# ajzhai/PEANUT

Measured on AMD Instinct MI355X. Metric: maps/sec for 480x480x(4+N_cat) prediction fwd, batch 32, higher is better.
Workload: dtype f32; 1 GPU; 480x480, 14-channel (4+10) partial maps -> 6-class prediction forward (PSPNet R50-V1c-D8), batch 32 per GPU, seeded random-init weights; survey_config=2, global_batch=32, parallelism=dp1 (map shards, no data-path collective)

## Files before the change

peanut_amd/csrc/conv_pw_ares.hip:

```cpp
#include <stdlib.h>

#include "common.h"
#include "conv_common.h"

namespace peanut {

namespace {

typedef const __attribute__((address_space(1))) void* gptr_t;
typedef __attribute__((address_space(3))) void* lptr_t;

__device__ __forceinline__ float load_uncounted(const float* ptr) {
  float v;
  asm volatile("global_load_dword %0, %1, off" : "=v"(v) : "v"(ptr) : "memory");
  return v;
}
template <int CH>
__device__ __forceinline__ void wait_uncounted(const float (&r)[CH], float a, float b) {
  static_assert(CH == 4 || CH == 8, "chunk of 4 or 8 values");
  __builtin_amdgcn_sched_barrier(0);
  if constexpr (CH == 4)
    asm volatile("s_waitcnt vmcnt(0)" ::"v"(r[0]), "v"(r[1]), "v"(r[2]), "v"(r[3]), "v"(a), "v"(b) : "memory");
  else
    asm volatile("s_waitcnt vmcnt(0)" ::"v"(r[0]), "v"(r[1]), "v"(r[2]), "v"(r[3]), "v"(r[4]), "v"(r[5]), "v"(r[6]), "v"(r[7]), "v"(a), "v"(b)
                 : "memory");
  __builtin_amdgcn_sched_barrier(0);
}

template <int NK, bool FLUSH>
__global__ __launch_bounds__(512) void conv_pw_ares_kernel(const ConvKParams p) {
  constexpr int BK = 32, K = NK * BK, TILE = 128 * BK;
  constexpr int CH = 32 / NK;
  static_assert(NK == 4 || NK == 8, "K = 128 or 256");
  __shared__ __attribute__((aligned(1024))) float smem[(NK + 2) * TILE];
  float* const bst = smem + NK * TILE;

  const int tid = threadIdx.x, lane = tid & 63;
  const int wave = __builtin_amdgcn_readfirstlane(tid >> 6);
  const int lr = lane >> 3, lp = lane & 7;
  const int wm = wave >> 2, wn = wave & 3;
  const int li = lane & 31, hi = lane >> 5;
  const bool late = p.phase_shift && wave >= 4;

  const int G = gridDim.x, bid = blockIdx.x;
  const int lw = (bid & 7) * (G >> 3) + (bid >> 3);
  const int NT = p.ntiles;
  const long long U = (long long)p.mtiles * NT;
  const int u0 = (int)(U * lw / G), u1 = (int)(U * (lw + 1) / G);
  if (u0 >= u1) return;

  const int pbn = p.ares_pbn;
  unsigned a_off[2], b_off[2];
#pragma unroll
  for (int j = 0; j < 2; ++j) {
    const int r = (wave * 2 + j) * 8 + lr;
    const int c = lp ^ ((r >> 1) & 7);
    a_off[j] = r * K + c * 4;
    b_off[j] = (r / pbn) * (NK * pbn * BK) + (r % pbn) * BK + c * 4;
  }
  auto dma_a = [&](int mt, int s) {
    const float* base = p.x + (size_t)mt * (128 * K) + s * BK;
#pragma unroll
    for (int j = 0; j < 2; ++j)
      __builtin_amdgcn_global_load_lds((gptr_t)(base + a_off[j]), (lptr_t)(smem + s * TILE + (wave * 2 + j) * 256), 16, 0, 0);
  };
  auto dma_b = [&](int mt, int nt, int kt, int stage) {
    const float* base = p.w + (p.mt_per_group ? (size_t)(mt / p.mt_per_group) * p.w_group_stride : 0) + (size_t)nt * (128 * K) + kt * (pbn * BK);
#pragma unroll
    for (int j = 0; j < 2; ++j)
      __builtin_amdgcn_global_load_lds((gptr_t)(base + b_off[j]), (lptr_t)(bst + stage * TILE + (wave * 2 + j) * 256), 16, 0, 0);
  };

  const int swz = (li >> 1) & 7;
  int sw[4];
#pragma unroll
  for (int ks = 0; ks < 4; ++ks) sw[ks] = ((ks * 2 + hi) ^ swz) * 4;
  const int a_row = (wm * 64 + li) * BK;
  const int b_row = (wn * 32 + li) * BK;

  f32x16 acc[2], acc2[2], prev[2];
#pragma unroll
  for (int t = 0; t < 2; ++t)
#pragma unroll
    for (int r = 0; r < 16; ++r) { acc[t][r] = 0.f; acc2[t][r] = 0.f; prev[t][r] = 0.f; }

  const size_t lane_el = (size_t)(wm * 64 + 4 * hi) * p.cout + wn * 32 + li;
  const bool has_res = p.res != nullptr;
  const size_t rstride = has_res ? (size_t)p.cout : 0;
  const size_t ostride = (size_t)p.cout;
  const float* res_run = has_res ? p.res + lane_el : p.zeros;
  float* out_run = p.y + lane_el;
  const float* prev_sc = p.scale + wn * 32 + li;
  const float* prev_sh = p.shift + wn * 32 + li;
  bool prev_valid = false;
  float scv = 1.f, shv = 0.f;
  const float alpha = p.alpha;
  const bool relu = p.relu != 0;

#define ARES_CHUNK_LOADS(kt)                                                              \
  float resv[CH];                                                                         \
  if ((kt) == 0) {                                                                        \
    scv = load_uncounted(prev_sc);                                                        \
    shv = load_uncounted(prev_sh);                                                        \
  }                                                                                       \
  _Pragma("unroll") for (int i = 0; i < CH; ++i)                                          \
    resv[i] = load_uncounted(res_run + (size_t)(8 * (i >> 2) + (i & 3)) * rstride);       \
  res_run += (size_t)(2 * CH) * rstride;
#define ARES_CHUNK_FINISH(kt)                                                             \
  if (prev_valid) {                                                   \
    _Pragma("unroll") for (int i = 0; i < CH; ++i) {                                      \
      const int idx = (kt) * CH + i;                                                      \
      float v = prev[idx >> 4][idx & 15] * (scv * alpha) + shv;                           \
      v += resv[i];                                                                       \
      if (relu) v = relu_keep_nan(v);                                                     \
      out_run[(size_t)(8 * (i >> 2) + (i & 3)) * ostride] = v;                            \
    }                                                                                     \
  }                                                                                       \
  out_run += (size_t)(2 * CH) * ostride;

  {
    const int mt = u0 / NT, nt = u0 - mt * NT;
#pragma unroll
    for (int s = 0; s < NK; ++s) dma_a(mt, s);
    dma_b(mt, nt, 0, 0);
    asm volatile("s_waitcnt vmcnt(0)" ::: "memory");
    __builtin_amdgcn_s_barrier();
    asm volatile("" ::: "memory");
  }

  int stage = 0;
  for (int u = u0; u < u1; ++u) {
    const int mt = u / NT, nt = u - mt * NT;
    const bool nxt = u + 1 < u1;
    const int mt_n = nxt ? (u + 1) / NT : mt;
    const int nt_n = nxt ? (u + 1) - mt_n * NT : 0;
    const bool refill_next = nxt && mt_n != mt;

    static_for<NK>([&](auto kc) {
      constexpr int kt = decltype(kc)::value;
      const float* const cur_b = bst + stage * TILE;
      const float* const cur_a = smem + kt * TILE;
      const bool more = (kt + 1 < NK) || nxt;
      ARES_CHUNK_LOADS(kt)
      auto request = [&]() {
        if (more) {
          if (kt + 1 < NK) dma_b(mt, nt, kt + 1, stage ^ 1);
          else dma_b(mt_n, nt_n, 0, stage ^ 1);
        }
      };
      if (!late) request();
      __builtin_amdgcn_sched_barrier(0);
      f32x4 af[4][2], bf[4];
#pragma unroll
      for (int j = 0; j < 4; ++j) {
        af[j][0] = *reinterpret_cast<const f32x4*>(cur_a + a_row + sw[j]);
        af[j][1] = *reinterpret_cast<const f32x4*>(cur_a + a_row + 32 * BK + sw[j]);
        bf[j] = *reinterpret_cast<const f32x4*>(cur_b + b_row + sw[j]);
      }
#pragma unroll
      for (int j = 0; j < 2; ++j)
#pragma unroll
        for (int kk = 0; kk < 4; ++kk)
#pragma unroll
          for (int t = 0; t < 2; ++t) acc[t] = __builtin_amdgcn_mfma_f32_32x32x2f32(af[j][t][kk], bf[j][kk], acc[t], 0, 0, 0);
      __builtin_amdgcn_sched_barrier(0);
      if (late) request();
      __builtin_amdgcn_sched_barrier(0);
#pragma unroll
      for (int j = 2; j < 4; ++j)
#pragma unroll
        for (int kk = 0; kk < 4; ++kk)
#pragma unroll
          for (int t = 0; t < 2; ++t) acc[t] = __builtin_amdgcn_mfma_f32_32x32x2f32(af[j][t][kk], bf[j][kk], acc[t], 0, 0, 0);
      if (FLUSH && (kt & 1)) {
#pragma unroll
        for (int t = 0; t < 2; ++t) {
          acc2[t] += acc[t];
#pragma unroll
          for (int r = 0; r < 16; ++r) acc[t][r] = 0.f;
        }
      }
      wait_uncounted<CH>(resv, scv, shv);
      ARES_CHUNK_FINISH(kt)
      if (kt >= 1) { if (refill_next) dma_a(mt_n, kt - 1); }
      asm volatile("s_waitcnt lgkmcnt(0)" ::: "memory");
      __builtin_amdgcn_s_barrier();
      asm volatile("" ::: "memory");
      stage ^= 1;
    });

#pragma unroll
    for (int t = 0; t < 2; ++t) {
      prev[t] = FLUSH ? acc2[t] : acc[t];
#pragma unroll
      for (int r = 0; r < 16; ++r) { acc[t][r] = 0.f; acc2[t][r] = 0.f; }
    }
    {
      const size_t unit_el = (size_t)mt * 128 * p.cout + (size_t)nt * 128 + lane_el;
      res_run = has_res ? p.res + unit_el : p.zeros;
      out_run = p.y + unit_el;
      const int ss_off = (p.mt_per_group && p.ss_group_stride) ? (mt / p.mt_per_group) * p.ss_group_stride : 0;
      prev_sc = p.scale + ss_off + nt * 128 + wn * 32 + li;
      prev_sh = p.shift + ss_off + nt * 128 + wn * 32 + li;
      prev_valid = true;
    }
    if (refill_next) dma_a(mt_n, NK - 1);
  }

  static_for<NK>([&](auto kc) {
    constexpr int kt = decltype(kc)::value;
    ARES_CHUNK_LOADS(kt)
    wait_uncounted<CH>(resv, scv, shv);
    ARES_CHUNK_FINISH(kt)
  });
#undef ARES_CHUNK_LOADS
#undef ARES_CHUNK_FINISH
}

template <int NK, bool FLUSH>
int launch_ares_t(ConvKParams p, hipStream_t stream) {
  const int cus = device_cus();
  if (cus < 8) return fail(-3, "conv_pw_ares: no current device");
  const long long U = (long long)p.mtiles * p.ntiles;
  long long G = U < cus ? U : cus;
  G -= G % 8;
  if (G < 8) return fail(-2, "conv_pw_ares: launch too small");
  hipLaunchKernelGGL((conv_pw_ares_kernel<NK, FLUSH>), dim3((unsigned)G), dim3(512), 0, stream, p);
  hipError_t e = hipGetLastError();
  if (e != hipSuccess) return fail(-3, std::string("conv_pw_ares launch: ") + hipGetErrorString(e));
  return 0;
}

}

bool conv_pw_uses_ares(int cin, int cout, long long M, int stride, bool two_source, int flush_ktiles, int bn_tile) {
  const bool on = opt(OPT_PW_ARES) != 0;
  const long long min_units = opt(OPT_PW_ARES_MINUNITS);
  if (!on || two_source || (cin != 128 && cin != 256) || stride != 1 || M % 128 != 0 || cout % 128 != 0) return false;
  if (bn_tile != 64 && bn_tile != 128) return false;
  if (flush_ktiles != 0 && flush_ktiles != 2) return false;
  return (M / 128) * (cout / 128) >= min_units;
}

int launch_conv_pw_ares(const ConvKParams& p0, int bn_tile, hipStream_t stream) {
  ConvKParams p = p0;
  p.phase_shift = opt(OPT_PW256_PHASE) != 0;
  p.ares_pbn = bn_tile;
  p.mtiles = p.M / 128;
  p.ntiles = p.cout / 128;
  const bool flush = p.flush == 2;
  if (p.c1 == 256) return flush ? launch_ares_t<8, true>(p, stream) : launch_ares_t<8, false>(p, stream);
  return flush ? launch_ares_t<4, true>(p, stream) : launch_ares_t<4, false>(p, stream);
}

}
```

peanut_amd/csrc/conv_pw256p.hip:

```cpp
#include <stdlib.h>

#include "common.h"
#include "conv_common.h"

namespace peanut {

namespace {

typedef const __attribute__((address_space(1))) void* gptr_t;
typedef __attribute__((address_space(3))) void* lptr_t;

__device__ __forceinline__ float p_load_uncounted(const float* base, unsigned byte_off) {
  float v;
  asm volatile("s_nop 4\n\tglobal_load_dword %0, %1, %2" : "=v"(v) : "v"(byte_off), "s"(base) : "memory");
  return v;
}
template <int N>
__device__ __forceinline__ void p_wait(const float (&r)[8], float a, float b, float c, float d) {
  __builtin_amdgcn_sched_barrier(0);
  if constexpr (N == 6)
    asm volatile("s_waitcnt vmcnt(6)" ::"v"(r[0]), "v"(r[1]), "v"(r[2]), "v"(r[3]), "v"(r[4]), "v"(r[5]), "v"(r[6]), "v"(r[7]), "v"(a), "v"(b),
                 "v"(c), "v"(d)
                 : "memory");
  else
    asm volatile("s_waitcnt vmcnt(0)" ::"v"(r[0]), "v"(r[1]), "v"(r[2]), "v"(r[3]), "v"(r[4]), "v"(r[5]), "v"(r[6]), "v"(r[7]), "v"(a), "v"(b),
                 "v"(c), "v"(d)
                 : "memory");
  __builtin_amdgcn_sched_barrier(0);
}

struct PItem { int mt, nt, kt0, kt1, part; };

template <bool RAGGED, bool FLUSH>
__global__ __launch_bounds__(512) void conv_pw_glds256p_kernel(const ConvKParams p) {
  constexpr int BM = 256, BN = 128, BK = 32, WN = 2;
  constexpr int A_FLOATS = BM * BK, B_FLOATS = BN * BK, STAGE = A_FLOATS + B_FLOATS;
  constexpr int A_INSTR = 4, B_INSTR = 2;
  __shared__ __attribute__((aligned(1024))) float smem[3 * STAGE + kMaxItems * 8];
  int* const plan = reinterpret_cast<int*>(smem + 3 * STAGE);

  const int tid = threadIdx.x, lane = tid & 63;
  const int wave = __builtin_amdgcn_readfirstlane(tid >> 6);
  const int lr = lane >> 3, lp = lane & 7;
  const int wm = wave / WN, wn = wave % WN;
  const int li = lane & 31, hi = lane >> 5;
  const bool late = p.phase_shift && wave >= 4;

  const int G = gridDim.x, bid = blockIdx.x;
  const int lw = (bid & 7) * (G >> 3) + (bid >> 3);
  const int nf = p.n_full / G;
  const int sp0 = (int)((long long)p.n_sp * lw / G), sp1 = (int)((long long)p.n_sp * (lw + 1) / G);
  const long long skU = p.sk_units;
  const int u0 = (skU > 0 && lw < p.sk_g) ? (int)(skU * lw / p.sk_g) : 0, u1 = (skU > 0 && lw < p.sk_g) ? (int)(skU * (lw + 1) / p.sk_g) : 0;
  const int upt = skU > 0 ? p.nkt / p.sk_q : 1;
  const int n_frag = u1 > u0 ? (u1 - 1) / upt - u0 / upt + 1 : 0;
  const int n_items = nf + (skU > 0 ? n_frag : sp1 - sp0);
  if (n_items == 0) return;
  if (n_items > kMaxItems) __builtin_trap();
  if (tid < n_items) {
    const int i = tid;
    PItem it;
    int tile;
    if (i >= nf && skU > 0) {
      const int j = u0 / upt + (i - nf);
      const int t0 = j * upt;
      it.kt0 = ((u0 > t0 ? u0 : t0) - t0) * p.sk_q;
      it.kt1 = ((u1 < t0 + upt ? u1 : t0 + upt) - t0) * p.sk_q;
      it.part = j * p.sk_maxp + (lw - sk_owner(skU, p.sk_g, (long long)t0));
      tile = p.n_full + j;
    } else if (i < nf) {
      tile = p.p_order ? (lw / (G >> 3)) * (nf * (G >> 3)) + i * (G >> 3) + lw % (G >> 3) : lw * nf + i;
      it.kt0 = 0; it.kt1 = p.nkt; it.part = -1;
    } else {
      const int s = sp0 + (i - nf);
      const int j = s / p.split_p, part = s - j * p.split_p;
      tile = p.n_full + j;
      it.part = s;
      it.kt0 = (int)((long long)part * p.nkt / p.split_p);
      it.kt1 = (int)((long long)(part + 1) * p.nkt / p.split_p);
    }
    tile_to_mn(p, tile, &it.mt, &it.nt);
    int* e = plan + i * 8;
    e[0] = it.mt; e[1] = it.nt; e[2] = it.kt0; e[3] = it.kt1; e[4] = it.part;
  }
  __syncthreads();
  auto item_at = [&](int i) {
    const int* e = plan + i * 8;
    PItem it;
    it.mt = __builtin_amdgcn_readfirstlane(e[0]);
    it.nt = __builtin_amdgcn_readfirstlane(e[1]);
    it.kt0 = __builtin_amdgcn_readfirstlane(e[2]);
    it.kt1 = __builtin_amdgcn_readfirstlane(e[3]);
    it.part = __builtin_amdgcn_readfirstlane(e[4]);
    return it;
  };

  unsigned a_pix[A_INSTR], a_chunk[A_INSTR], b_off[B_INSTR];
#pragma unroll
  for (int j = 0; j < A_INSTR; ++j) {
    const int r = (wave * A_INSTR + j) * 8 + lr;
    a_chunk[j] = (unsigned)((lp ^ ((r >> 1) & 7)) * 16);
    a_pix[j] = 0;
  }
#pragma unroll
  for (int j = 0; j < B_INSTR; ++j) {
    const int r = (wave * B_INSTR + j) * 8 + lr;
    b_off[j] = (unsigned)(r * BK * 4 + (lp ^ ((r >> 1) & 7)) * 16);
  }
  int d_item = 0, d_left = 0, d_kt = 0;
  const float* d_wtile = p.w;
  auto cursor_open = [&](int i) {
    const PItem it = item_at(i);
    const int m0 = it.mt * BM;
#pragma unroll
    for (int j = 0; j < A_INSTR; ++j) {
      int m = m0 + (wave * A_INSTR + j) * 8 + lr;
      if (RAGGED) m = m < p.M ? m : p.M - 1;
      const int b = m / p.HoWo;
      const int rem = m - b * p.HoWo;
      const int oy = rem / p.Wo, ox = rem - oy * p.Wo;
      a_pix[j] = (unsigned)(b * p.H * p.W + oy * p.stride * p.W + ox * p.stride);
    }
    d_wtile = p.w + (p.mt_per_group ? (size_t)(it.mt / p.mt_per_group) * p.w_group_stride : 0) + (size_t)it.nt * p.nkt * (BN * BK);
    d_kt = it.kt0;
    d_left = it.kt1 - it.kt0;
  };
  const int k1 = p.c1 / BK;
  auto request = [&](float* stage) {
    const bool live = d_left > 0;
    if (!live) --d_kt;
    const bool second = d_kt >= k1;
    const char* abase = reinterpret_cast<const char*>(second ? p.x2 : p.x) + (size_t)(second ? d_kt - k1 : d_kt) * (BK * 4);
    const unsigned cbytes = (unsigned)(second ? p.c2 : p.c1) * 4u;
#pragma unroll
    for (int j = 0; j < A_INSTR; ++j)
      __builtin_amdgcn_global_load_lds((gptr_t)(abase + (a_pix[j] * cbytes + a_chunk[j])), (lptr_t)(stage + (wave * A_INSTR + j) * 256), 16, 0, 0);
    const char* bbase = reinterpret_cast<const char*>(d_wtile + (size_t)d_kt * (BN * BK));
#pragma unroll
    for (int j = 0; j < B_INSTR; ++j)
      __builtin_amdgcn_global_load_lds((gptr_t)(bbase + b_off[j]), (lptr_t)(stage + A_FLOATS + (wave * B_INSTR + j) * 256), 16, 0, 0);
    ++d_kt;
    if (live) --d_left;
  };
  auto cursor_advance = [&]() {
    if (d_left == 0 && d_item + 1 < n_items) {
      ++d_item;
      cursor_open(d_item);
    }
  };

  const int swz = (li >> 1) & 7;
  int sw[4];
#pragma unroll
  for (int ks = 0; ks < 4; ++ks) sw[ks] = ((ks * 2 + hi) ^ swz) * 4;
  const int a_row = (wm * 64 + li) * BK;
  const int b_row = A_FLOATS + (wn * 64 + li) * BK;

  f32x16 acc[2][2], prev[2][2], acc2[2][2];
#pragma unroll
  for (int t = 0; t < 2; ++t)
#pragma unroll
    for (int u = 0; u < 2; ++u)
#pragma unroll
      for (int r = 0; r < 16; ++r) { acc[t][u][r] = 0.f; prev[t][u][r] = 0.f; acc2[t][u][r] = 0.f; }
#define P256_PREV(t, u, r) (FLUSH ? acc2[t][u][r] : prev[t][u][r])
#define P256_FLUSH_STEP()                                                                                 \
  if (FLUSH) {                                                                                            \
    _Pragma("unroll") for (int t = 0; t < 2; ++t)                                                         \
      _Pragma("unroll") for (int u = 0; u < 2; ++u) {                                                     \
        acc2[t][u] += acc[t][u];                                                                          \
        _Pragma("unroll") for (int r = 0; r < 16; ++r) acc[t][u][r] = 0.f;                                \
      }                                                                                                   \
  }

  const int cout = p.cout;
  bool prev_valid = false, prev_raw = false;
  const float* prev_res = p.zeros;
  float* prev_out = p.y;
  const float* prev_ss = p.scale;
  unsigned prev_rs = 0;
  unsigned prev_os = (unsigned)cout * 4;
  int prev_rows = BM;
  const unsigned lane_row = (unsigned)(wm * 64 + 4 * hi), lane_col = (unsigned)(wn * 64 + li);
  const unsigned ss_lane = lane_col * 4;
  const unsigned shift_delta = (unsigned)((p.shift - p.scale) * 4);
  float sc0 = 1.f, sc1 = 1.f, sh0 = 0.f, sh1 = 0.f;
  const bool has_res = p.res != nullptr;
  const float alpha = p.alpha;
  const bool relu = p.relu != 0;

#define P256_EPI_SS_LOADS()                                                                                       \
  {                                                                                                               \
    sc0 = p_load_uncounted(prev_ss, ss_lane);                                                                     \
    sc1 = p_load_uncounted(prev_ss, ss_lane + 128);                                                               \
    sh0 = p_load_uncounted(prev_ss, ss_lane + shift_delta);                                                       \
    sh1 = p_load_uncounted(prev_ss, ss_lane + shift_delta + 128);                                                 \
  }
#define P256_EPI_LOADS(c)                                                                                         \
  float resv[8];                                                                                                  \
  {                                                                                                               \
    if ((c) == 0) {                                                                                               \
      sc0 = p_load_uncounted(prev_ss, ss_lane);                                                                   \
      sc1 = p_load_uncounted(prev_ss, ss_lane + 128);                                                             \
      sh0 = p_load_uncounted(prev_ss, ss_lane + shift_delta);                                                     \
      sh1 = p_load_uncounted(prev_ss, ss_lane + shift_delta + 128);                                               \
    }                                                                                                             \
    const unsigned lane_off = (lane_row * prev_rs) + (prev_rs ? lane_col * 4 : 0);                                \
                                                      \
    int row_limit = prev_rows - 1;                                                                                \
    if (RAGGED) asm volatile("" : "+s"(row_limit));                                                               \
    _Pragma("unroll") for (int i = 0; i < 8; ++i) {                                                               \
      const int r = ((c) & 1) * 8 + i, row = ((c) >> 2) * 32 + (r & 3) + 8 * (r >> 2);                            \
      unsigned roff = lane_off + (unsigned)row * prev_rs;                                                         \
      if (RAGGED) {                                                                                               \
        const int rr = (int)lane_row + row;                                                                       \
                                           \
        roff = __umul24((unsigned)(rr < row_limit ? rr : row_limit), prev_rs) + (prev_rs ? lane_col * 4 : 0);     \
      }                                                                                                           \
      resv[i] = p_load_uncounted(prev_res, roff + (prev_rs ? (((c) >> 1) & 1) * 128u : 0u));                      \
    }                                                                                                             \
  }
#define P256_EPI_FINISH(c) P256_EPI_FINISH_RV(c, resv)
#define P256_EPI_FINISH_RV(c, RV)                                                                                 \
  if (prev_valid) {                                                                                               \
    const float scv = (((c) >> 1) & 1) ? sc1 : sc0, shv = (((c) >> 1) & 1) ? sh1 : sh0;                           \
    char* const obase = reinterpret_cast<char*>(prev_out) + (lane_row * prev_os + lane_col * 4 + (((c) >> 1) & 1) * 128u); \
    _Pragma("unroll") for (int i = 0; i < 8; ++i) {                                                               \
      const int r = ((c) & 1) * 8 + i, row = ((c) >> 2) * 32 + (r & 3) + 8 * (r >> 2);                            \
      float v = P256_PREV((c) >> 2, ((c) >> 1) & 1, r);                                                           \
      if (!prev_raw) {                                                                                            \
        v = v * (scv * alpha) + shv;                                                                              \
        v += RV[i];                                                                                               \
        if (relu) v = relu_keep_nan(v);                                                                           \
      }                                                                                                           \
      if (!RAGGED || (int)lane_row + row < prev_rows) *reinterpret_cast<float*>(obase + (unsigned)row * prev_os) = v; \
    }                                                                                                             \
  }

  cursor_open(0);
  request(smem);
  cursor_advance();
  request(smem + STAGE);
  cursor_advance();
  asm volatile("s_waitcnt vmcnt(6)" ::: "memory");
  asm volatile("s_waitcnt lgkmcnt(0)" ::: "memory");
  __builtin_amdgcn_s_barrier();
  asm volatile("" ::: "memory");
  int o_cur = 0, o_mid = STAGE, o_fill = 2 * STAGE;

#define P256_MFMA_PAIR()                                                                                  \
  _Pragma("unroll") for (int j = 0; j < 2; ++j)                                                           \
    _Pragma("unroll") for (int kk = 0; kk < 4; ++kk)                                                      \
      _Pragma("unroll") for (int t = 0; t < 2; ++t)                                                       \
        _Pragma("unroll") for (int u = 0; u < 2; ++u)                                                     \
          acc[t][u] = __builtin_amdgcn_mfma_f32_32x32x2f32(af[j][t][kk], bf[j][u][kk], acc[t][u], 0, 0, 0);
#define P256_READ_PAIR(g)                                                                                            \
  _Pragma("unroll") for (int j = 0; j < 2; ++j) {                                                                    \
    _Pragma("unroll") for (int t = 0; t < 2; ++t) af[j][t] = *reinterpret_cast<const f32x4*>(cur + a_row + t * 32 * BK + sw[(g) + j]); \
    _Pragma("unroll") for (int u = 0; u < 2; ++u) bf[j][u] = *reinterpret_cast<const f32x4*>(cur + b_row + u * 32 * BK + sw[(g) + j]); \
  }
#define P256_ITERATION()                                                                                  \
  {                                                                                                       \
    const float* const cur = smem + o_cur;                                                                \
    float* const fill = smem + o_fill;                                                                    \
    float resv_none[8] = {0.f, 0.f, 0.f, 0.f, 0.f, 0.f, 0.f, 0.f};                                        \
    (void)resv_none;                                                                                      \
    P256_EPI_LOADS_IF                                                                                     \
    if (!late) request(fill);                                                                             \
    __builtin_amdgcn_sched_barrier(0);                                                                    \
    f32x4 af[2][2], bf[2][2];                                                                             \
    P256_READ_PAIR(0);                                                                                    \
    P256_MFMA_PAIR();                                                                                     \
    __builtin_amdgcn_sched_barrier(0);                                                                    \
    if (late) request(fill);                                                                              \
    __builtin_amdgcn_sched_barrier(0);                                                                    \
    P256_READ_PAIR(2);                                                                                    \
    P256_MFMA_PAIR();                                                                                     \
    p_wait<6>(P256_RESV, sc0, sc1, sh0, sh1);                                                             \
    P256_EPI_FINISH_IF                                                                                    \
    P256_FLUSH_IF                                                                                         \
    cursor_advance();                                                                                     \
    asm volatile("s_waitcnt lgkmcnt(0)" ::: "memory");                                                    \
    __builtin_amdgcn_s_barrier();                                                                         \
    asm volatile("" ::: "memory");                                                                        \
    { const int tmp = o_cur; o_cur = o_mid; o_mid = o_fill; o_fill = tmp; }                               \
  }

  for (int ci = 0; ci < n_items; ++ci) {
    const PItem it = item_at(ci);
    const int nk = it.kt1 - it.kt0;
    static_for<8>([&](auto kc) {
      constexpr int c = decltype(kc)::value;
      if (c < nk) {
        if constexpr (!FLUSH) {
#define P256_EPI_LOADS_IF P256_EPI_LOADS(c)
#define P256_EPI_FINISH_IF P256_EPI_FINISH(c)
#define P256_FLUSH_IF
#define P256_RESV resv
          P256_ITERATION()
#undef P256_EPI_LOADS_IF
#undef P256_EPI_FINISH_IF
#undef P256_FLUSH_IF
#undef P256_RESV
        } else {
#define P256_EPI_LOADS_IF if (c == 0) P256_EPI_SS_LOADS()
#define P256_EPI_FINISH_IF                                                                   \
  if (c == 0) { P256_EPI_FINISH_RV(0, resv_none) P256_EPI_FINISH_RV(1, resv_none) P256_EPI_FINISH_RV(2, resv_none) P256_EPI_FINISH_RV(3, resv_none) } \
  if (c == 1) {                                                                              \
    P256_EPI_FINISH_RV(4, resv_none) P256_EPI_FINISH_RV(5, resv_none) P256_EPI_FINISH_RV(6, resv_none) P256_EPI_FINISH_RV(7, resv_none) \
    _Pragma("unroll") for (int t = 0; t < 2; ++t)                                            \
      _Pragma("unroll") for (int u = 0; u < 2; ++u)                                          \
        _Pragma("unroll") for (int r = 0; r < 16; ++r) acc2[t][u][r] = 0.f;                  \
  }
#define P256_FLUSH_IF if (c & 1) { P256_FLUSH_STEP() }
#define P256_RESV resv_none
          P256_ITERATION()
#undef P256_EPI_LOADS_IF
#undef P256_EPI_FINISH_IF
#undef P256_FLUSH_IF
#undef P256_RESV
        }
      }
    });
    for (int kt = 8; kt < nk; ++kt) {
#define P256_EPI_LOADS_IF
#define P256_EPI_FINISH_IF
#define P256_FLUSH_IF if (kt & 1) { P256_FLUSH_STEP() }
#define P256_RESV resv_none
      P256_ITERATION()
#undef P256_EPI_LOADS_IF
#undef P256_EPI_FINISH_IF
#undef P256_FLUSH_IF
#undef P256_RESV
    }
    if (FLUSH && (nk & 1)) { P256_FLUSH_STEP() }
    if (!FLUSH && nk < 8 && prev_valid) {
      static_for<8>([&](auto kc) {
        constexpr int c = decltype(kc)::value;
        if (c >= nk) {
          P256_EPI_LOADS(c)
          p_wait<0>(resv, sc0, sc1, sh0, sh1);
          P256_EPI_FINISH(c)
        }
      });
    }
    if (!FLUSH) {
#pragma unroll
      for (int t = 0; t < 2; ++t)
#pragma unroll
        for (int u = 0; u < 2; ++u) {
          prev[t][u] = acc[t][u];
#pragma unroll
          for (int r = 0; r < 16; ++r) acc[t][u][r] = 0.f;
        }
    }
    {
      const size_t tile_el = (size_t)it.mt * BM * cout + (size_t)it.nt * BN;
      prev_valid = true;
      prev_raw = it.part >= 0;
      prev_rows = BM;
      if (prev_raw) {
        prev_out = p.partial + (size_t)it.part * (BM * BN);
        prev_os = BN * 4;
        prev_res = p.zeros;
        prev_rs = 0;
      } else {
        if (RAGGED && p.M - it.mt * BM < BM) prev_rows = p.M - it.mt * BM;
        prev_out = p.y + tile_el;
        prev_os = (unsigned)cout * 4;
        prev_res = has_res ? p.res + tile_el : p.zeros;
        prev_rs = has_res ? (unsigned)cout * 4 : 0;
      }
      prev_ss = p.scale + ((p.mt_per_group && p.ss_group_stride) ? (it.mt / p.mt_per_group) * p.ss_group_stride : 0) + it.nt * BN;
    }
  }
  static_for<8>([&](auto kc) {
    constexpr int c = decltype(kc)::value;
    P256_EPI_LOADS(c)
    p_wait<0>(resv, sc0, sc1, sh0, sh1);
    P256_EPI_FINISH(c)
  });
  asm volatile("s_waitcnt vmcnt(0)" ::: "memory");
#undef P256_PREV
#undef P256_FLUSH_STEP
#undef P256_EPI_SS_LOADS
#undef P256_EPI_FINISH_RV
#undef P256_ITERATION
#undef P256_READ_PAIR
#undef P256_MFMA_PAIR
#undef P256_EPI_LOADS
#undef P256_EPI_FINISH
}

}

bool conv_pw_uses_256p(int cout, long long M, int mt_per_group, int bn_tile, int cin, int flush_ktiles, long long in_pixels) {
  const int min_k = (int)opt(OPT_PW256P_MINK);
  if (min_k <= 0 || bn_tile != 128 || cin < min_k || cin < 256) return false;
  if (flush_ktiles != 0 && (flush_ktiles != 2 || cin > opt(OPT_PW256P_FLUSH))) return false;
  if (mt_per_group % 2 != 0) return false;
  if (cout % 128 != 0) return false;
  const long long in_rows = in_pixels > M ? in_pixels : M;
  if (in_rows * (long long)cin * 4 >= (1LL << 32) || M * (long long)cout * 4 >= (1LL << 32)) return false;
  return ((M + 255) / 256) * (cout / 128) >= opt(OPT_PW256P_MINTILES);
}

int launch_conv_pw256p(const ConvKParams& p0, const ConvRoute& r, float* ws, hipStream_t stream) {
  ConvKParams p = p0;
  const PersistentPlan& pl = r.plan;
  if (!pl.scratch_ok) return fail(-2, "conv_pw256p: split-K scratch too small");
  const int G = r.G;
  const int mtiles = (p.M + 255) / 256;
  const int t = mtiles * p.ntiles - pl.n_full;
  p.split_p = pl.split_p; p.n_sp = pl.n_sp; p.n_full = pl.n_full;
  p.sk_units = pl.sk_units; p.sk_maxp = pl.sk_maxp; p.sk_g = pl.sk_g; p.sk_q = pl.sk_q;
  p.partial = ws;
  p.mtiles = mtiles;
  p.nchunk = (int)opt(OPT_NCHUNK);
  p.phase_shift = opt(OPT_PW256_PHASE) != 0;
  p.p_order = opt(OPT_PW256P_ORDER) != 0;
  if (p.mt_per_group) p.mt_per_group /= 2;
  const bool ragged = p.M % 256 != 0;
  if (p.flush) {
    if (ragged) hipLaunchKernelGGL((conv_pw_glds256p_kernel<true, true>), dim3((unsigned)G), dim3(512), 0, stream, p);
    else hipLaunchKernelGGL((conv_pw_glds256p_kernel<false, true>), dim3((unsigned)G), dim3(512), 0, stream, p);
  } else {
    if (ragged) hipLaunchKernelGGL((conv_pw_glds256p_kernel<true, false>), dim3((unsigned)G), dim3(512), 0, stream, p);
    else hipLaunchKernelGGL((conv_pw_glds256p_kernel<false, false>), dim3((unsigned)G), dim3(512), 0, stream, p);
  }
  if (p.n_sp > 0 || p.sk_units > 0)
    hipLaunchKernelGGL((conv_splitk_reduce_kernel<256, 128>), dim3((unsigned)t, 256 / 16), dim3(256), 0, stream, p);
  hipError_t e = hipGetLastError();
  if (e != hipSuccess) return fail(-3, std::string("conv_pw256p launch: ") + hipGetErrorString(e));
  return 0;
}

}
```

Before: 891.2 maps/s.

## Deepen weight prefetch ring, use partial vmcnt waits, and defer epilogue stores

Replaces the two-stage weight double buffer with a three-slot ring so B tiles are fetched two k-steps ahead. For K=256 the last A slice is moved into a ring slot to save shared memory. Waits on residual loads now use a nonzero vmcnt, so in-flight DMA is not drained at every chunk. Epilogue stores are deferred by one chunk and addressed through SGPR base plus VGPR offset. A peeled first unit removes the prev_valid branch. The aim is to hide global-load latency behind MFMA work, at the cost of fragile hand-counted vmcnt values and an added s_nop before each load.

```diff
diff --git a/peanut_amd/csrc/conv_pw_ares.hip b/peanut_amd/csrc/conv_pw_ares.hip
--- a/peanut_amd/csrc/conv_pw_ares.hip
+++ b/peanut_amd/csrc/conv_pw_ares.hip
@@ -10,19 +10,21 @@
 typedef const __attribute__((address_space(1))) void* gptr_t;
 typedef __attribute__((address_space(3))) void* lptr_t;
 
-__device__ __forceinline__ float load_uncounted(const float* ptr) {
+__device__ __forceinline__ float load_uncounted(const float* base, unsigned byte_off) {
   float v;
-  asm volatile("global_load_dword %0, %1, off" : "=v"(v) : "v"(ptr) : "memory");
+  asm volatile("s_nop 4\n\tglobal_load_dword %0, %1, %2" : "=v"(v) : "v"(byte_off), "s"(base) : "memory");
   return v;
 }
-template <int CH>
+template <int N, int CH>
 __device__ __forceinline__ void wait_uncounted(const float (&r)[CH], float a, float b) {
   static_assert(CH == 4 || CH == 8, "chunk of 4 or 8 values");
+  static_assert(N >= 0 && N < 64, "vmcnt is a 6-bit counter");
   __builtin_amdgcn_sched_barrier(0);
   if constexpr (CH == 4)
-    asm volatile("s_waitcnt vmcnt(0)" ::"v"(r[0]), "v"(r[1]), "v"(r[2]), "v"(r[3]), "v"(a), "v"(b) : "memory");
+    asm volatile("s_waitcnt vmcnt(%6)" ::"v"(r[0]), "v"(r[1]), "v"(r[2]), "v"(r[3]), "v"(a), "v"(b), "n"(N) : "memory");
   else
-    asm volatile("s_waitcnt vmcnt(0)" ::"v"(r[0]), "v"(r[1]), "v"(r[2]), "v"(r[3]), "v"(r[4]), "v"(r[5]), "v"(r[6]), "v"(r[7]), "v"(a), "v"(b)
+    asm volatile("s_waitcnt vmcnt(%10)" ::"v"(r[0]), "v"(r[1]), "v"(r[2]), "v"(r[3]), "v"(r[4]), "v"(r[5]), "v"(r[6]), "v"(r[7]), "v"(a), "v"(b),
+                 "n"(N)
                  : "memory");
   __builtin_amdgcn_sched_barrier(0);
 }
@@ -32,8 +34,9 @@
   constexpr int BK = 32, K = NK * BK, TILE = 128 * BK;
   constexpr int CH = 32 / NK;
   static_assert(NK == 4 || NK == 8, "K = 128 or 256");
-  __shared__ __attribute__((aligned(1024))) float smem[(NK + 2) * TILE];
-  float* const bst = smem + NK * TILE;
+  constexpr int NA = NK == 8 ? NK - 1 : NK;
+  __shared__ __attribute__((aligned(1024))) float smem[(NA + 3) * TILE];
+  float* const ring = smem + NA * TILE;
 
   const int tid = threadIdx.x, lane = tid & 63;
   const int wave = __builtin_amdgcn_readfirstlane(tid >> 6);
@@ -55,20 +58,29 @@
   for (int j = 0; j < 2; ++j) {
     const int r = (wave * 2 + j) * 8 + lr;
     const int c = lp ^ ((r >> 1) & 7);
-    a_off[j] = r * K + c * 4;
-    b_off[j] = (r / pbn) * (NK * pbn * BK) + (r % pbn) * BK + c * 4;
+    a_off[j] = (unsigned)(r * K + c * 4) * 4u;
+    b_off[j] = (unsigned)((r / pbn) * (NK * pbn * BK) + (r % pbn) * BK + c * 4) * 4u;
   }
-  auto dma_a = [&](int mt, int s) {
-    const float* base = p.x + (size_t)mt * (128 * K) + s * BK;
-#pragma unroll
-    for (int j = 0; j < 2; ++j)
-      __builtin_amdgcn_global_load_lds((gptr_t)(base + a_off[j]), (lptr_t)(smem + s * TILE + (wave * 2 + j) * 256), 16, 0, 0);
+  auto dma_a = [&](int mt, int s, float* dst) {
+    const char* base = reinterpret_cast<const char*>(p.x + (size_t)mt * (128 * K) + s * BK);
+    asm volatile("" : "+s"(base));
+#pragma unroll
+    for (int j = 0; j < 2; ++j) {
+      unsigned off = a_off[j];
+      asm volatile("" : "+v"(off));
+      __builtin_amdgcn_global_load_lds((gptr_t)(base + off), (lptr_t)(dst + (wave * 2 + j) * 256), 16, 0, 0);
+    }
   };
-  auto dma_b = [&](int mt, int nt, int kt, int stage) {
-    const float* base = p.w + (p.mt_per_group ? (size_t)(mt / p.mt_per_group) * p.w_group_stride : 0) + (size_t)nt * (128 * K) + kt * (pbn * BK);
-#pragma unroll
-    for (int j = 0; j < 2; ++j)
-      __builtin_amdgcn_global_load_lds((gptr_t)(base + b_off[j]), (lptr_t)(bst + stage * TILE + (wave * 2 + j) * 256), 16, 0, 0);
+  auto dma_b = [&](int mt, int nt, int kt, float* dst) {
+    const char* base = reinterpret_cast<const char*>(p.w + (p.mt_per_group ? (size_t)(mt / p.mt_per_group) * p.w_group_stride : 0) +
+                                                     (size_t)nt * (128 * K) + kt * (pbn * BK));
+    asm volatile("" : "+s"(base));
+#pragma unroll
+    for (int j = 0; j < 2; ++j) {
+      unsigned off = b_off[j];
+      asm volatile("" : "+v"(off));
+      __builtin_amdgcn_global_load_lds((gptr_t)(base + off), (lptr_t)(dst + (wave * 2 + j) * 256), 16, 0, 0);
+    }
   };
 
   const int swz = (li >> 1) & 7;
@@ -84,52 +96,65 @@
 #pragma unroll
     for (int r = 0; r < 16; ++r) { acc[t][r] = 0.f; acc2[t][r] = 0.f; prev[t][r] = 0.f; }
 
-  const size_t lane_el = (size_t)(wm * 64 + 4 * hi) * p.cout + wn * 32 + li;
   const bool has_res = p.res != nullptr;
-  const size_t rstride = has_res ? (size_t)p.cout : 0;
-  const size_t ostride = (size_t)p.cout;
-  const float* res_run = has_res ? p.res + lane_el : p.zeros;
-  float* out_run = p.y + lane_el;
-  const float* prev_sc = p.scale + wn * 32 + li;
-  const float* prev_sh = p.shift + wn * 32 + li;
-  bool prev_valid = false;
+  const unsigned os = (unsigned)p.cout * 4u;
+  const unsigned rs = has_res ? os : 0u;
+  const unsigned ss_lane = (unsigned)(wn * 32 + li) * 4u;
+  const unsigned lane_b = (unsigned)(wm * 64 + 4 * hi) * os + ss_lane;
+  const unsigned res_lane = has_res ? lane_b : 0u;
+  const float* res_tile = has_res ? p.res : p.zeros;
+  float* out_tile = p.y;
+  const float* prev_sc = p.scale;
+  const float* prev_sh = p.shift;
   float scv = 1.f, shv = 0.f;
   const float alpha = p.alpha;
   const bool relu = p.relu != 0;
 
+#define ARES_ROW(c, i) (2 * CH * (c) + 8 * ((i) >> 2) + ((i) & 3))
 #define ARES_CHUNK_LOADS(kt)                                                              \
   float resv[CH];                                                                         \
   if ((kt) == 0) {                                                                        \
-    scv = load_uncounted(prev_sc);                                                        \
-    shv = load_uncounted(prev_sh);                                                        \
+    scv = load_uncounted(prev_sc, ss_lane);                                               \
+    shv = load_uncounted(prev_sh, ss_lane);                                               \
   }                                                                                       \
+                                                         \
+  unsigned rs_c = rs;                                                                     \
+  asm volatile("" : "+s"(rs_c));                                                          \
   _Pragma("unroll") for (int i = 0; i < CH; ++i)                                          \
-    resv[i] = load_uncounted(res_run + (size_t)(8 * (i >> 2) + (i & 3)) * rstride);       \
-  res_run += (size_t)(2 * CH) * rstride;
+    resv[i] = load_uncounted(reinterpret_cast<const float*>(reinterpret_cast<const char*>(res_tile) + (size_t)ARES_ROW(kt, i) * rs_c), res_lane);
 #define ARES_CHUNK_FINISH(kt)                                                             \
-  if (prev_valid) {                                                   \
-    _Pragma("unroll") for (int i = 0; i < CH; ++i) {                                      \
-      const int idx = (kt) * CH + i;                                                      \
-      float v = prev[idx >> 4][idx & 15] * (scv * alpha) + shv;                           \
-      v += resv[i];                                                                       \
-      if (relu) v = relu_keep_nan(v);                                                     \
-      out_run[(size_t)(8 * (i >> 2) + (i & 3)) * ostride] = v;                            \
-    }                                                                                     \
-  }                                                                                       \
-  out_run += (size_t)(2 * CH) * ostride;
+  _Pragma("unroll") for (int i = 0; i < CH; ++i) {                                        \
+    const int idx = (kt) * CH + i;                                                        \
+    float v = prev[idx >> 4][idx & 15] * (scv * alpha) + shv;                             \
+    v += resv[i];                                                                         \
+    if (relu) v = relu_keep_nan(v);                                                       \
+    prev[idx >> 4][idx & 15] = v;                                                         \
+  }
+#define ARES_CHUNK_STORE(c)                                                               \
+  unsigned os_c = os;                                                                     \
+  asm volatile("" : "+s"(os_c));                                                          \
+  _Pragma("unroll") for (int i = 0; i < CH; ++i) {                                        \
+    const int idx = (c) * CH + i;                                                         \
+    char* const row = reinterpret_cast<char*>(out_tile) + (size_t)ARES_ROW(c, i) * os_c;  \
+    *reinterpret_cast<float*>(row + lane_b) = prev[idx >> 4][idx & 15];                   \
+  }
 
   {
     const int mt = u0 / NT, nt = u0 - mt * NT;
 #pragma unroll
-    for (int s = 0; s < NK; ++s) dma_a(mt, s);
-    dma_b(mt, nt, 0, 0);
+    for (int s = 0; s < NA; ++s) dma_a(mt, s, smem + s * TILE);
+    dma_b(mt, nt, 0, ring);
+    if constexpr (NK == 4) dma_b(mt, nt, 1, ring + TILE);
     asm volatile("s_waitcnt vmcnt(0)" ::: "memory");
     __builtin_amdgcn_s_barrier();
     asm volatile("" ::: "memory");
   }
 
-  int stage = 0;
-  for (int u = u0; u < u1; ++u) {
+  int o_cur = 0, o_mid = TILE, o_fill = 2 * TILE;
+  bool refill_prev = false;
+  auto run_unit = [&](auto first_c, const int u) {
+    constexpr bool FIRST = decltype(first_c)::value != 0;
+    constexpr int SN = FIRST ? 0 : CH;
     const int mt = u / NT, nt = u - mt * NT;
     const bool nxt = u + 1 < u1;
     const int mt_n = nxt ? (u + 1) / NT : mt;
@@ -138,17 +163,35 @@
 
     static_for<NK>([&](auto kc) {
       constexpr int kt = decltype(kc)::value;
-      const float* const cur_b = bst + stage * TILE;
-      const float* const cur_a = smem + kt * TILE;
-      const bool more = (kt + 1 < NK) || nxt;
+      const float* const cur_b = ring + (NK == 8 ? (kt % 3) * TILE : o_cur);
+      const float* const cur_a = (NK == 8 && kt == 7) ? ring + 2 * TILE : smem + kt * TILE;
+      if constexpr (kt >= 1) {
+        if (refill_next) dma_a(mt_n, kt - 1, smem + (kt - 1) * TILE);
+      } else if constexpr (NK == 4) {
+        if (refill_prev) dma_a(mt, NK - 1, smem + (NK - 1) * TILE);
+      }
       ARES_CHUNK_LOADS(kt)
-      auto request = [&]() {
-        if (more) {
-          if (kt + 1 < NK) dma_b(mt, nt, kt + 1, stage ^ 1);
-          else dma_b(mt_n, nt_n, 0, stage ^ 1);
+      auto issue = [&]() {
+        if constexpr (NK == 8) {
+          if constexpr (kt == 0) {
+            dma_b(mt, nt, 1, ring + TILE);
+            dma_b(mt, nt, 2, ring + 2 * TILE);
+          } else if constexpr (kt <= 5) {
+            dma_b(mt, nt, kt + 2, ring + ((kt + 2) % 3) * TILE);
+          } else if constexpr (kt == 6) {
+            dma_a(mt, 7, ring + 2 * TILE);
+          } else {
+            dma_b(mt_n, nt_n, 0, ring);
+          }
+        } else {
+          if constexpr (kt + 2 < NK) dma_b(mt, nt, kt + 2, ring + o_fill);
+          else dma_b(mt_n, nt_n, kt + 2 - NK, ring + o_fill);
         }
+        if constexpr (!FIRST && kt >= 1) { ARES_CHUNK_STORE(kt - 1) }
       };
-      if (!late) request();
+      constexpr bool DUE_NEXT = NK == 8 && (kt == 0 || kt >= 6);
+      const bool late_k = late && !DUE_NEXT;
+      if (!late_k) issue();
       __builtin_amdgcn_sched_barrier(0);
       f32x4 af[4][2], bf[4];
 #pragma unroll
@@ -164,7 +207,7 @@
 #pragma unroll
           for (int t = 0; t < 2; ++t) acc[t] = __builtin_amdgcn_mfma_f32_32x32x2f32(af[j][t][kk], bf[j][kk], acc[t], 0, 0, 0);
       __builtin_amdgcn_sched_barrier(0);
-      if (late) request();
+      if (late_k) issue();
       __builtin_amdgcn_sched_barrier(0);
 #pragma unroll
       for (int j = 2; j < 4; ++j)
@@ -180,13 +223,16 @@
           for (int r = 0; r < 16; ++r) acc[t][r] = 0.f;
         }
       }
-      wait_uncounted<CH>(resv, scv, shv);
-      ARES_CHUNK_FINISH(kt)
-      if (kt >= 1) { if (refill_next) dma_a(mt_n, kt - 1); }
+      constexpr int WN = (NK == 8 ? (kt == 0 ? 2 : kt <= 5 ? 2 + SN : SN) : (kt == 0 ? 2 : 2 + SN));
+      wait_uncounted<WN, CH>(resv, scv, shv);
+      if constexpr (!FIRST) {
+        ARES_CHUNK_FINISH(kt)
+        if constexpr (kt == NK - 1) { ARES_CHUNK_STORE(kt) }
+      }
       asm volatile("s_waitcnt lgkmcnt(0)" ::: "memory");
       __builtin_amdgcn_s_barrier();
       asm volatile("" ::: "memory");
-      stage ^= 1;
+      if constexpr (NK == 4) { const int tmp = o_cur; o_cur = o_mid; o_mid = o_fill; o_fill = tmp; }
     });
 
 #pragma unroll
@@ -196,25 +242,30 @@
       for (int r = 0; r < 16; ++r) { acc[t][r] = 0.f; acc2[t][r] = 0.f; }
     }
     {
-      const size_t unit_el = (size_t)mt * 128 * p.cout + (size_t)nt * 128 + lane_el;
-      res_run = has_res ? p.res + unit_el : p.zeros;
-      out_run = p.y + unit_el;
+      const size_t tile_el = (size_t)mt * 128 * p.cout + (size_t)nt * 128;
+      res_tile = has_res ? p.res + tile_el : p.zeros;
+      out_tile = p.y + tile_el;
       const int ss_off = (p.mt_per_group && p.ss_group_stride) ? (mt / p.mt_per_group) * p.ss_group_stride : 0;
-      prev_sc = p.scale + ss_off + nt * 128 + wn * 32 + li;
-      prev_sh = p.shift + ss_off + nt * 128 + wn * 32 + li;
-      prev_valid = true;
+      prev_sc = p.scale + ss_off + nt * 128;
+      prev_sh = p.shift + ss_off + nt * 128;
     }
-    if (refill_next) dma_a(mt_n, NK - 1);
-  }
+    refill_prev = refill_next;
+  };
+
+  run_unit(IC<1>{}, u0);
+  for (int u = u0 + 1; u < u1; ++u) run_unit(IC<0>{}, u);
 
   static_for<NK>([&](auto kc) {
     constexpr int kt = decltype(kc)::value;
     ARES_CHUNK_LOADS(kt)
-    wait_uncounted<CH>(resv, scv, shv);
+    wait_uncounted<0, CH>(resv, scv, shv);
     ARES_CHUNK_FINISH(kt)
+    ARES_CHUNK_STORE(kt)
   });
 #undef ARES_CHUNK_LOADS
 #undef ARES_CHUNK_FINISH
+#undef ARES_CHUNK_STORE
+#undef ARES_ROW
 }
 
 template <int NK, bool FLUSH>
```

After: 896.2 maps/s, median of 6. About the same (+0.6%).

## Split ares tiles at half-unit granularity and pipeline 256p epilogue residual drain

Applied to the files above, without the earlier changes.

The ares kernel now divides work among workgroups in half-tile units, so a boundary tile is shared by two workgroups. Each owner computes and stores only its own half: waves whose M half falls outside the range skip the MFMAs but still take part in DMA and barriers. In the 256p kernel, the non-ragged epilogue drain now issues residual loads for four chunks before waiting on each in turn, and skips residual loads when the output is raw. This targets load imbalance across CUs and serialized load-wait latency in the tail drain, at the cost of extra code paths and idle waves on boundary tiles.

```diff
diff --git a/peanut_amd/csrc/ares_ranges.h b/peanut_amd/csrc/ares_ranges.h
--- /dev/null
+++ b/peanut_amd/csrc/ares_ranges.h
@@ -0,0 +1,20 @@
+#pragma once
+
+namespace peanut {
+
+struct AresRange {
+  long long h0, h1;
+  int u0, u1;
+};
+
+constexpr AresRange ares_range(long long U, int G, int lw) {
+  const long long H = 2 * U, h0 = H * lw / G, h1 = H * (lw + 1) / G;
+  return AresRange{h0, h1, (int)(h0 >> 1), (int)((h1 + 1) >> 1)};
+}
+
+constexpr bool ares_owns(const AresRange& r, int u, int part) {
+  const long long h = 2LL * u + part;
+  return h >= r.h0 && h < r.h1;
+}
+
+}
diff --git a/peanut_amd/csrc/conv_pw256p.hip b/peanut_amd/csrc/conv_pw256p.hip
--- a/peanut_amd/csrc/conv_pw256p.hip
+++ b/peanut_amd/csrc/conv_pw256p.hip
@@ -28,6 +28,21 @@
                  : "memory");
   __builtin_amdgcn_sched_barrier(0);
 }
+#define P256_WAIT_LANDS(N)                                                                                                              \
+  asm volatile("s_waitcnt vmcnt(" #N ") ; lands %0 %1 %2 %3 %4 %5 %6 %7 %8 %9 %10 %11" ::"v"(r[0]), "v"(r[1]), "v"(r[2]), "v"(r[3]), "v"(r[4]), \
+               "v"(r[5]), "v"(r[6]), "v"(r[7]), "v"(a), "v"(b), "v"(c), "v"(d)                                                         \
+               : "memory")
+template <int N>
+__device__ __forceinline__ void p_wait_lands(const float (&r)[8], float a, float b, float c, float d) {
+  static_assert(N == 24 || N == 16 || N == 8 || N == 0, "groups of eight");
+  __builtin_amdgcn_sched_barrier(0);
+  if constexpr (N == 24) P256_WAIT_LANDS(24);
+  else if constexpr (N == 16) P256_WAIT_LANDS(16);
+  else if constexpr (N == 8) P256_WAIT_LANDS(8);
+  else P256_WAIT_LANDS(0);
+  __builtin_amdgcn_sched_barrier(0);
+}
+#undef P256_WAIT_LANDS
 
 struct PItem { int mt, nt, kt0, kt1, part; };
 
@@ -196,10 +211,11 @@
     sh0 = p_load_uncounted(prev_ss, ss_lane + shift_delta);                                                       \
     sh1 = p_load_uncounted(prev_ss, ss_lane + shift_delta + 128);                                                 \
   }
-#define P256_EPI_LOADS(c)                                                                                         \
-  float resv[8];                                                                                                  \
-  {                                                                                                               \
-    if ((c) == 0) {                                                                                               \
+#define P256_EPI_LOADS(c) P256_EPI_LOADS_RV(c, resv, true)
+#define P256_EPI_LOADS_RV(c, RV, SS)                                                                              \
+  float RV[8];                                                                                                    \
+  {                                                                                                            \
+    if ((SS) && (c) == 0) {                                                                                       \
       sc0 = p_load_uncounted(prev_ss, ss_lane);                                                                   \
       sc1 = p_load_uncounted(prev_ss, ss_lane + 128);                                                             \
       sh0 = p_load_uncounted(prev_ss, ss_lane + shift_delta);                                                     \
@@ -217,18 +233,19 @@
                                            \
         roff = __umul24((unsigned)(rr < row_limit ? rr : row_limit), prev_rs) + (prev_rs ? lane_col * 4 : 0);     \
       }                                                                                                           \
-      resv[i] = p_load_uncounted(prev_res, roff + (prev_rs ? (((c) >> 1) & 1) * 128u : 0u));                      \
+      RV[i] = p_load_uncounted(prev_res, roff + (prev_rs ? (((c) >> 1) & 1) * 128u : 0u));                        \
     }                                                                                                             \
   }
 #define P256_EPI_FINISH(c) P256_EPI_FINISH_RV(c, resv)
-#define P256_EPI_FINISH_RV(c, RV)                                                                                 \
+#define P256_EPI_FINISH_RV(c, RV) P256_EPI_FINISH_RAW(c, RV, prev_raw)
+#define P256_EPI_FINISH_RAW(c, RV, RAW)                                                                           \
   if (prev_valid) {                                                                                               \
     const float scv = (((c) >> 1) & 1) ? sc1 : sc0, shv = (((c) >> 1) & 1) ? sh1 : sh0;                           \
     char* const obase = reinterpret_cast<char*>(prev_out) + (lane_row * prev_os + lane_col * 4 + (((c) >> 1) & 1) * 128u); \
     _Pragma("unroll") for (int i = 0; i < 8; ++i) {                                                               \
       const int r = ((c) & 1) * 8 + i, row = ((c) >> 2) * 32 + (r & 3) + 8 * (r >> 2);                            \
       float v = P256_PREV((c) >> 2, ((c) >> 1) & 1, r);                                                           \
-      if (!prev_raw) {                                                                                            \
+      if (!(RAW)) {                                                                                               \
         v = v * (scv * alpha) + shv;                                                                              \
         v += RV[i];                                                                                               \
         if (relu) v = relu_keep_nan(v);                                                                           \
@@ -236,6 +253,38 @@
       if (!RAGGED || (int)lane_row + row < prev_rows) *reinterpret_cast<float*>(obase + (unsigned)row * prev_os) = v; \
     }                                                                                                             \
   }
+
+#define P256_DRAIN_HALF(c0, W1, W2, W3, FIRST, SS)                                                                \
+  {                                                                                                               \
+    P256_EPI_LOADS_RV((c0), rv0, SS)                                                                              \
+    P256_EPI_LOADS_RV((c0) + 1, rv1, false)                                                                       \
+    P256_EPI_LOADS_RV((c0) + 2, rv2, false)                                                                       \
+    P256_EPI_LOADS_RV((c0) + 3, rv3, false)                                                                       \
+    p_wait_lands<24>(rv0, sc0, sc1, sh0, sh1);                                                                    \
+    if ((c0) >= (FIRST)) { P256_EPI_FINISH_RAW((c0), rv0, false) }                                                \
+    p_wait_lands<W1>(rv1, sc0, sc1, sh0, sh1);                                                                    \
+    if ((c0) + 1 >= (FIRST)) { P256_EPI_FINISH_RAW((c0) + 1, rv1, false) }                                        \
+    p_wait_lands<W2>(rv2, sc0, sc1, sh0, sh1);                                                                    \
+    if ((c0) + 2 >= (FIRST)) { P256_EPI_FINISH_RAW((c0) + 2, rv2, false) }                                        \
+    p_wait_lands<W3>(rv3, sc0, sc1, sh0, sh1);                                                                    \
+    if ((c0) + 3 >= (FIRST)) { P256_EPI_FINISH_RAW((c0) + 3, rv3, false) }                                        \
+  }
+#define P256_DRAIN_SERIAL(FIRST)                                                                                  \
+  static_for<8>([&](auto kc) {                                                                                    \
+    constexpr int c = decltype(kc)::value;                                                                        \
+    if (c >= (FIRST)) {                                                                                           \
+      P256_EPI_LOADS(c)                                                                                           \
+      p_wait<0>(resv, sc0, sc1, sh0, sh1);                                                                        \
+      P256_EPI_FINISH(c)                                                                                          \
+    }                                                                                                             \
+  });
+#define P256_DRAIN_RAW(FIRST)                                                                                     \
+  static_for<8>([&](auto kc) {                                                                                    \
+    constexpr int c = decltype(kc)::value;                                                                        \
+    const float rv_none[8] = {0.f, 0.f, 0.f, 0.f, 0.f, 0.f, 0.f, 0.f};                                            \
+    (void)rv_none;                                                                                                \
+    if (c >= (FIRST)) { P256_EPI_FINISH_RAW(c, rv_none, true) }                                                   \
+  });
 
   cursor_open(0);
   request(smem);
@@ -335,14 +384,14 @@
     }
     if (FLUSH && (nk & 1)) { P256_FLUSH_STEP() }
     if (!FLUSH && nk < 8 && prev_valid) {
-      static_for<8>([&](auto kc) {
-        constexpr int c = decltype(kc)::value;
-        if (c >= nk) {
-          P256_EPI_LOADS(c)
-          p_wait<0>(resv, sc0, sc1, sh0, sh1);
-          P256_EPI_FINISH(c)
-        }
-      });
+      if constexpr (RAGGED) {
+        P256_DRAIN_SERIAL(nk)
+      } else if (prev_raw) {
+        P256_DRAIN_RAW(nk)
+      } else {
+        if (nk < 4) P256_DRAIN_HALF(0, 16, 8, 0, nk, false)
+        P256_DRAIN_HALF(4, 16, 8, 0, nk, false)
+      }
     }
     if (!FLUSH) {
 #pragma unroll
@@ -374,12 +423,14 @@
       prev_ss = p.scale + ((p.mt_per_group && p.ss_group_stride) ? (it.mt / p.mt_per_group) * p.ss_group_stride : 0) + it.nt * BN;
     }
   }
-  static_for<8>([&](auto kc) {
-    constexpr int c = decltype(kc)::value;
-    P256_EPI_LOADS(c)
-    p_wait<0>(resv, sc0, sc1, sh0, sh1);
-    P256_EPI_FINISH(c)
-  });
+  if constexpr (RAGGED) {
+    P256_DRAIN_SERIAL(0)
+  } else if (prev_raw) {
+    P256_DRAIN_RAW(0)
+  } else {
+    P256_DRAIN_HALF(0, 24, 24, 24, 0, true)
+    P256_DRAIN_HALF(4, 24, 24, 24, 0, false)
+  }
   asm volatile("s_waitcnt vmcnt(0)" ::: "memory");
 #undef P256_PREV
 #undef P256_FLUSH_STEP
@@ -389,7 +440,12 @@
 #undef P256_READ_PAIR
 #undef P256_MFMA_PAIR
 #undef P256_EPI_LOADS
+#undef P256_EPI_LOADS_RV
 #undef P256_EPI_FINISH
+#undef P256_EPI_FINISH_RAW
+#undef P256_DRAIN_HALF
+#undef P256_DRAIN_SERIAL
+#undef P256_DRAIN_RAW
 }
 
 }
diff --git a/peanut_amd/csrc/conv_pw_ares.hip b/peanut_amd/csrc/conv_pw_ares.hip
--- a/peanut_amd/csrc/conv_pw_ares.hip
+++ b/peanut_amd/csrc/conv_pw_ares.hip
@@ -1,5 +1,6 @@
 #include <stdlib.h>
 
+#include "ares_ranges.h"
 #include "common.h"
 #include "conv_common.h"
 
@@ -26,6 +27,8 @@
                  : "memory");
   __builtin_amdgcn_sched_barrier(0);
 }
+template <bool B>
+struct BC { static constexpr bool value = B; };
 
 template <int NK, bool FLUSH>
 __global__ __launch_bounds__(512) void conv_pw_ares_kernel(const ConvKParams p) {
@@ -46,8 +49,10 @@
   const int lw = (bid & 7) * (G >> 3) + (bid >> 3);
   const int NT = p.ntiles;
   const long long U = (long long)p.mtiles * NT;
-  const int u0 = (int)(U * lw / G), u1 = (int)(U * (lw + 1) / G);
+  const AresRange range = ares_range(U, G, lw);
+  const int u0 = range.u0, u1 = range.u1;
   if (u0 >= u1) return;
+  const int my_h0 = (int)range.h0 - wm, my_h1 = (int)range.h1 - wm;
 
   const int pbn = p.ares_pbn;
   unsigned a_off[2], b_off[2];
@@ -135,66 +140,77 @@
     const int mt_n = nxt ? (u + 1) / NT : mt;
     const int nt_n = nxt ? (u + 1) - mt_n * NT : 0;
     const bool refill_next = nxt && mt_n != mt;
-
-    static_for<NK>([&](auto kc) {
-      constexpr int kt = decltype(kc)::value;
-      const float* const cur_b = bst + stage * TILE;
-      const float* const cur_a = smem + kt * TILE;
-      const bool more = (kt + 1 < NK) || nxt;
-      ARES_CHUNK_LOADS(kt)
-      auto request = [&]() {
-        if (more) {
-          if (kt + 1 < NK) dma_b(mt, nt, kt + 1, stage ^ 1);
-          else dma_b(mt_n, nt_n, 0, stage ^ 1);
-        }
-      };
-      if (!late) request();
-      __builtin_amdgcn_sched_barrier(0);
-      f32x4 af[4][2], bf[4];
-#pragma unroll
-      for (int j = 0; j < 4; ++j) {
-        af[j][0] = *reinterpret_cast<const f32x4*>(cur_a + a_row + sw[j]);
-        af[j][1] = *reinterpret_cast<const f32x4*>(cur_a + a_row + 32 * BK + sw[j]);
-        bf[j] = *reinterpret_cast<const f32x4*>(cur_b + b_row + sw[j]);
+    const bool mine = 2 * u >= my_h0 && 2 * u < my_h1;
+
+    auto k_loop = [&](auto mine_c) {
+      constexpr bool MINE = decltype(mine_c)::value;
+      static_for<NK>([&](auto kc) {
+        constexpr int kt = decltype(kc)::value;
+        const float* const cur_b = bst + stage * TILE;
+        const float* const cur_a = smem + kt * TILE;
+        const bool more = (kt + 1 < NK) || nxt;
+        ARES_CHUNK_LOADS(kt)
+        auto request = [&]() {
+          if (more) {
+            if (kt + 1 < NK) dma_b(mt, nt, kt + 1, stage ^ 1);
+            else dma_b(mt_n, nt_n, 0, stage ^ 1);
+          }
+        };
+        if (!late) request();
+        __builtin_amdgcn_sched_barrier(0);
+        f32x4 af[4][2], bf[4];
+        if constexpr (MINE) {
+#pragma unroll
+          for (int j = 0; j < 4; ++j) {
+            af[j][0] = *reinterpret_cast<const f32x4*>(cur_a + a_row + sw[j]);
+            af[j][1] = *reinterpret_cast<const f32x4*>(cur_a + a_row + 32 * BK + sw[j]);
+            bf[j] = *reinterpret_cast<const f32x4*>(cur_b + b_row + sw[j]);
+          }
+#pragma unroll
+          for (int j = 0; j < 2; ++j)
+#pragma unroll
+            for (int kk = 0; kk < 4; ++kk)
+#pragma unroll
+              for (int t = 0; t < 2; ++t) acc[t] = __builtin_amdgcn_mfma_f32_32x32x2f32(af[j][t][kk], bf[j][kk], acc[t], 0, 0, 0);
+        }
+        __builtin_amdgcn_sched_barrier(0);
+        if (late) request();
+        __builtin_amdgcn_sched_barrier(0);
+        if constexpr (MINE) {
+#pragma unroll
+          for (int j = 2; j < 4; ++j)
+#pragma unroll
+            for (int kk = 0; kk < 4; ++kk)
+#pragma unroll
+              for (int t = 0; t < 2; ++t) acc[t] = __builtin_amdgcn_mfma_f32_32x32x2f32(af[j][t][kk], bf[j][kk], acc[t], 0, 0, 0);
+        }
+        if (MINE && FLUSH && (kt & 1)) {
+#pragma unroll
+          for (int t = 0; t < 2; ++t) {
+            acc2[t] += acc[t];
+#pragma unroll
+            for (int r = 0; r < 16; ++r) acc[t][r] = 0.f;
+          }
+        }
+        wait_uncounted<CH>(resv, scv, shv);
+        ARES_CHUNK_FINISH(kt)
+        if (kt >= 1) { if (refill_next) dma_a(mt_n, kt - 1); }
+        asm volatile("s_waitcnt lgkmcnt(0)" ::: "memory");
+        __builtin_amdgcn_s_barrier();
+        asm volatile("" ::: "memory");
+        stage ^= 1;
+      });
+      if constexpr (MINE) {
+#pragma unroll
+        for (int t = 0; t < 2; ++t) {
+          prev[t] = FLUSH ? acc2[t] : acc[t];
+#pragma unroll
+          for (int r = 0; r < 16; ++r) { acc[t][r] = 0.f; acc2[t][r] = 0.f; }
+        }
       }
-#pragma unroll
-      for (int j = 0; j < 2; ++j)
-#pragma unroll
-        for (int kk = 0; kk < 4; ++kk)
-#pragma unroll
-          for (int t = 0; t < 2; ++t) acc[t] = __builtin_amdgcn_mfma_f32_32x32x2f32(af[j][t][kk], bf[j][kk], acc[t], 0, 0, 0);
-      __builtin_amdgcn_sched_barrier(0);
-      if (late) request();
-      __builtin_amdgcn_sched_barrier(0);
-#pragma unroll
-      for (int j = 2; j < 4; ++j)
-#pragma unroll
-        for (int kk = 0; kk < 4; ++kk)
-#pragma unroll
-          for (int t = 0; t < 2; ++t) acc[t] = __builtin_amdgcn_mfma_f32_32x32x2f32(af[j][t][kk], bf[j][kk], acc[t], 0, 0, 0);
-      if (FLUSH && (kt & 1)) {
-#pragma unroll
-        for (int t = 0; t < 2; ++t) {
-          acc2[t] += acc[t];
-#pragma unroll
-          for (int r = 0; r < 16; ++r) acc[t][r] = 0.f;
-        }
-      }
-      wait_uncounted<CH>(resv, scv, shv);
-      ARES_CHUNK_FINISH(kt)
-      if (kt >= 1) { if (refill_next) dma_a(mt_n, kt - 1); }
-      asm volatile("s_waitcnt lgkmcnt(0)" ::: "memory");
-      __builtin_amdgcn_s_barrier();
-      asm volatile("" ::: "memory");
-      stage ^= 1;
-    });
-
-#pragma unroll
-    for (int t = 0; t < 2; ++t) {
-      prev[t] = FLUSH ? acc2[t] : acc[t];
-#pragma unroll
-      for (int r = 0; r < 16; ++r) { acc[t][r] = 0.f; acc2[t][r] = 0.f; }
-    }
+    };
+    if (__builtin_expect(mine, true)) k_loop(BC<true>{});
+    else k_loop(BC<false>{});
     {
       const size_t unit_el = (size_t)mt * 128 * p.cout + (size_t)nt * 128 + lane_el;
       res_run = has_res ? p.res + unit_el : p.zeros;
@@ -202,7 +218,7 @@
       const int ss_off = (p.mt_per_group && p.ss_group_stride) ? (mt / p.mt_per_group) * p.ss_group_stride : 0;
       prev_sc = p.scale + ss_off + nt * 128 + wn * 32 + li;
       prev_sh = p.shift + ss_off + nt * 128 + wn * 32 + li;
-      prev_valid = true;
+      prev_valid = mine;
     }
     if (refill_next) dma_a(mt_n, NK - 1);
   }
```

After: 886.9 maps/s before, 886.4 maps/s after. About the same (-0.1%).
